# Validation-m3sSAGE/GCN_Recommendation

Measured on AMD Instinct MI355X. Metric: propagated edges/sec (SpMM) + Recall@20, Amazon-Books 3-layer d=64, higher is better.
Workload: dtype f32; 1 GPU; C3 full Amazon-Books-2023 shape (10.3M users x 4.4M items x 29.5M interactions); generator=powerlaw, users=10300000, items=4400000, interactions=29500000, nnz=56305746, d=64, layers=3, brands=0, content_dim=0, hub_threshold=128, hub_mode=exact, emu_min_degree=1024, parallelism=single

## Files before the change

### gcn_recommendation_amd/csrc/lgcn_engine.hip

```cpp
#include "lgcn_kernels.h"

#include <string.h>
#include <algorithm>
#include <functional>
#include <new>
#include <vector>

namespace lgcn_detail {
int g_rows_per_group = 0;
int g_unroll = 0;
int g_mean_prefetch = 0;
int g_min_groups = 0;
int g_emu_margin = (128 << 4) | 4;
int g_sample_blocks = 0;
int g_fusion_bwd_blocks = 0;
}

namespace {
__global__ void k_coo_inspect(const int64_t* __restrict__ rows, const int64_t* __restrict__ cols,
                              int64_t nnz, int32_t n_rows, int32_t n_cols, int32_t* flags) {
    const int64_t j = (int64_t)blockIdx.x * blockDim.x + threadIdx.x;
    if (j >= nnz) return;
    const int64_t r = rows[j], c = cols[j];
    int f = 0;
// ... 355 lines not shown

int scale_rows(const lgcn_rows_t& x, int32_t n_rows, int32_t d, float div, float* y, int64_t ldy,
               hipStream_t s) {
    const bool vec_ok = rows_aligned(x) && al16(y) && (ldy % 4 == 0);
    const Geo g = pick_geo(d, vec_ok);
    ScaleF f{&x, n_rows, g.dW, div, y, ldy, s};
    return dispatch_geo(g, f);
}

struct MeanEmptyF {
    const int32_t* row_ids; int32_t n; const lgcn_rows_t* e0; int32_t dW; float div;
    int32_t inv_bits; float* y; int64_t ldy; hipStream_t s;
    template <typename V, int G, int NV> int operator()() const {
        return launch_mean_empty_t<V, G, NV>(row_ids, n, *e0, dW, div, inv_bits, y, ldy, s);
    }
};

int mean_empty(const int32_t* row_ids, int32_t n, const lgcn_epilogue_t& ep_in, float* y,
               int64_t ldy, int32_t d, hipStream_t s) {
    const lgcn_epilogue_t ep = with_pow2(ep_in);
    const bool vec_ok = rows_aligned(ep.prev0) && al16(y) && (ldy % 4 == 0);
    const Geo g = pick_geo(d, vec_ok);
    MeanEmptyF f{row_ids, n, &ep.prev0, g.dW, ep.div, ep.pad, y, ldy, s};
    return dispatch_geo(g, f);
}

lgcn_rows_t dense_rows(const float* p, int32_t n, int64_t ld) {
    lgcn_rows_t r;
    r.p0 = r.p1 = r.p2 = p;
    r.end0 = r.end1 = n;
    r.ld = ld;
    return r;
}

int valid_geom(int32_t n_rows, int32_t d) {
    if (n_rows < 0 || d < 1 || d > 2048) return LGCN_EINVAL;
    return 0;
}

}

template <typename V>
__global__ __launch_bounds__(256) void k_add_nonzero(const V* __restrict__ src, V* __restrict__ dst,
                                                     int64_t m) {
    for (int64_t i = (int64_t)blockIdx.x * 256 + threadIdx.x; i < m;
         i += (int64_t)gridDim.x * 256) {
// ... 598 lines not shown
}

int link(const lgcn_sched* sc, hipStream_t from, hipStream_t to) {
    hipEvent_t e;
    if (int r = ev_next(sc, &e)) return r;
    if (int r = herr(hipEventRecord(e, from))) return r;
    return herr(hipStreamWaitEvent(to, e, 0));
}

int record(const lgcn_sched* sc, hipStream_t st, hipEvent_t* out) {
    if (int r = ev_next(sc, out)) return r;
    return herr(hipEventRecord(*out, st));
}

int wait_ev(hipStream_t st, hipEvent_t e) { return e ? herr(hipStreamWaitEvent(st, e, 0)) : 0; }

struct Deps {
    hipEvent_t late[3] = {nullptr, nullptr, nullptr};
    hipEvent_t late_emu[2] = {nullptr, nullptr};
    hipEvent_t part_wait[2] = {nullptr, nullptr};
    bool defer = false;
    hipEvent_t part_done[2] = {nullptr, nullptr};
    hipStream_t lk = nullptr;
};

int wait_late(hipStream_t st, const Deps* dp, bool emu = true) {
    if (!dp) return 0;
    for (hipEvent_t e : dp->late)
        if (int r = wait_ev(st, e)) return r;
    if (emu)
        for (hipEvent_t e : dp->late_emu)
            if (int r = wait_ev(st, e)) return r;
    return 0;
}

int part_blocks(const lgcn_edge_t* edges, const lgcn_hub_plan_t& p, const EmuPart& q,
                const lgcn_rows_t& x, float xdiv, const uint32_t* x_nz, int32_t d,
                const lgcn_emu_row_t* live, hipStream_t s) {
    if (q.b1 <= q.b0) return 0;
    const int64_t b0 = q.b0;
    return lgcn_emu_blocks(edges, p.emu_blocks + b0, q.b1 - q.b0, x, xdiv, x_nz, d,
                           p.emu_rel + b0 * d * LGCN_EMU_CANDS,
                           static_cast<char*>(p.emu_meta) + b0 * d * LGCN_EMU_META_BYTES,
                           p.emu_stage ? p.emu_stage + b0 * (d + 1) * LGCN_EMU_BLOCK : nullptr,
                           live, s);
}

// ... 10 lines not shown
bool chain_ok(const lgcn_rows_t& x, int32_t d) {
    return lgcn_chain_supported(d) && x.ld % 4 == 0 && al16(x.p0) && al16(x.p1) && al16(x.p2);
}

int plan_layer(const int32_t* rowptr, const lgcn_edge_t* edges, const int32_t* row_ids,
               int32_t n, const lgcn_hub_plan_t& p, const lgcn_rows_t& x, float xdiv,
               const uint32_t* x_nz, float* y, int64_t ldy, int32_t d, const lgcn_epilogue_t& ep,
               const lgcn_sched* sc, hipStream_t s, Deps* dp = nullptr) {
    const int32_t ne = p.n_emu_rows;
    const bool live = x_nz && p.emu_live && ne > 0 && chain_ok(x, d) && (!sc || sc->chain);
    const bool chains = !live && ne > p.emu_part_rows[1] && chain_ok(x, d) && (!sc || sc->chain);
    if ((chains || live ? p.emu_part_blocks[1] : p.n_emu_blocks) > p.emu_scratch_blocks)
        return LGCN_EINVAL;
    hipEvent_t* tr = sc ? sc->trace : nullptr;
    auto mark = [&](int k, hipStream_t st) -> int {
        return tr && tr[k] ? herr(hipEventRecord(tr[k], st)) : 0;
    };
    const EmuPart parts[3] = {{0, p.emu_part_rows[0], 0, p.emu_part_blocks[0]},
                              {p.emu_part_rows[0], p.emu_part_rows[1], p.emu_part_blocks[0],
                               p.emu_part_blocks[1]},
                              {p.emu_part_rows[1], ne, p.emu_part_blocks[1], p.n_emu_blocks}};
    const int slots[3] = {sc ? sc->slots[0] : 0, sc ? sc->slots[1] : 0, sc ? sc->slots[1] : 0};
    auto layer_kernel = [&](hipStream_t st) -> int {
        if (sc && sc->t0)
            if (int e = herr(hipEventRecord(sc->t0, st))) return e;
        if (int e = spmm_layer(rowptr, edges, row_ids, n, p.threshold, p.items, p.n_items,
                               p.partials, x, y, ldy, d, ep, xdiv, x_nz, st))
            return e;
        if (sc && sc->t1)
            if (int e = herr(hipEventRecord(sc->t1, st))) return e;
        return hub_combine(p.rows, p.n_rows, p.n_pre, p.partials, y, ldy, d, ep, st);
    };
    const bool has_late = dp && (dp->late[0] || dp->late[1] || dp->late[2] ||
                                 dp->late_emu[0] || dp->late_emu[1]);
    const bool defer_epi = sc && has_late && ep.mode == LGCN_EPI_MEAN && p.emu_out && ne > 0 &&
                           !live;
    lgcn_epilogue_t ep_rows;
    memset(&ep_rows, 0, sizeof(ep_rows));
    ep_rows.mode = LGCN_EPI_ROWS;
    auto emu_y = [&](int i) { return defer_epi ? p.emu_out + (int64_t)parts[i].r0 * d : y; };
    const int64_t emu_ld = defer_epi ? d : ldy;
    const lgcn_epilogue_t& emu_ep = defer_epi ? ep_rows : ep;
    auto chain_rows = [&](hipStream_t st) -> int {
        const EmuPart& q = parts[2];
        if (q.r1 <= q.r0) return 0;
        return lgcn_chain_rows(edges, p.emu_blocks, p.emu_rows + q.r0, q.r1 - q.r0, x, xdiv,
                               emu_y(2), emu_ld, d, &emu_ep, st);
    };
    const lgcn_emu_row_t* lflags =
        live ? lgcn_live_flags(p.emu_live, ne, p.n_emu_blocks) : nullptr;
    auto live_rows = [&](hipStream_t st) -> int {
        return lgcn_live_rows(edges, p.emu_blocks, p.n_emu_blocks, p.emu_rows, ne, x, xdiv, x_nz,
                              y, ldy, d, &ep, p.emu_part_rows[1], LGCN_LIVE_MAX, p.emu_live, st);
    };
// ... 208 lines not shown
    return 0;
}

bool classes_hold(const lgcn_sides_t& sd, const lgcn_hub_plan_t* plans) {
    for (int j = 0; j < 2; ++j) {
        const lgcn_hub_plan_t& p = plans[2 * 3 + j];
        if (p.emu_part_rows[0] > sd.part_rows[0] || p.emu_part_rows[1] > sd.part_rows[1])
            return false;
    }
    return true;
}

struct LayerIO {
    lgcn_rows_t x;
    float xdiv;
    const uint32_t* x_nz;
    float* y;
    lgcn_epilogue_t ep;
};

int seg_layer(const int32_t* rowptr, const lgcn_edge_t* edges, const int32_t* row_ids,
              int32_t lo, int32_t hi, const lgcn_hub_plan_t* plans, int k, int g,
              const LayerIO& io, int32_t d, const lgcn_sched* sc, const Lane& L, Deps* dp,
              int32_t empty_tail = 0) {
    if (empty_tail > 0) {
        hi -= empty_tail;
        if (io.ep.mode == LGCN_EPI_MEAN)
            if (int e = mean_empty(row_ids + hi, empty_tail, io.ep, io.y, d, d, L.main)) return e;
    }
    if (hi <= lo) {
        if (dp && dp->defer && sc)
            for (int i = 0; i < 2; ++i)
                if (int e = record(sc, L.main, &dp->part_done[i])) return e;
        return 0;
    }
    const int h = (k - 1) * kSegs + g;
    lgcn_sched v;
    const lgcn_sched* vp = nullptr;
    if (L.view) {
        v = *L.view;
        v.t0 = sc->timing_sides ? sc->timing_sides[2 * h] : nullptr;
        v.t1 = sc->timing_sides ? sc->timing_sides[2 * h + 1] : nullptr;
        v.trace = sc->trace_sides ? sc->trace_sides + h * 8 : nullptr;
        vp = &v;
    }
    Deps local;
    Deps* dq = dp;
    if (!vp && dp && dp->defer && sc) {
        local = *dp;
        local.defer = false;
        dq = &local;
    }
    if (int e = plan_layer(rowptr + lo, edges, row_ids + lo, hi - lo, plans[2 * g + (k & 1)],
                           io.x, io.xdiv, io.x_nz, io.y, d, d, io.ep, vp, L.main, dq))
        return e;
    if (dq == &local)
        for (int i = 0; i < 2; ++i)
            if (int e = record(sc, L.main, &dp->part_done[i])) return e;
    return 0;
}

int run_sides(const int32_t* rowptr, const lgcn_edge_t* edges, const int32_t* row_ids,
              const lgcn_sides_t& sd, const lgcn_hub_plan_t* plans, int32_t d, int32_t K,
              const std::function<LayerIO(int)>& layer, const lgcn_sched* sched, hipStream_t s,
              const int32_t* empty_tail = nullptr) {
    Lane lanes[2];
    bool l1_aux = false;
    if (sched) sched->pool->next = 0;
    const bool two = make_lanes(sched, s, lanes, l1_aux);
    const bool cap = capture_restricted(s);
    const bool classes = sched && sched->classes && classes_hold(sd, plans) && !cap;
    if (sched) sched->pool->state[3] = classes ? 1 : 0;
    const int32_t lo[kSegs] = {0, sd.class_end[0], sd.class_end[1], sd.split};
    const int32_t hi[kSegs] = {sd.class_end[0], sd.class_end[1], sd.split, 0};
    auto seg_hi = [&](int g, int32_t n) { return g == 3 ? n : hi[g]; };
    const int32_t n = sd.n;
    if (int e = fork_lanes(sched, two, lanes[1], s)) return e;
    constexpr int KM = LGCN_MAX_LAYERS + 2;
    hipEvent_t cls[KM][3] = {}, ab[KM] = {}, rest[KM] = {}, part[KM][2] = {};
    for (int k = 1; k <= K; ++k) {
        const LayerIO io = layer(k);
        const bool mean = io.ep.mode == LGCN_EPI_MEAN;
        {
            const Lane& L = lanes[(k + 1 + K) & 1];
            Deps dp;
            if (classes && k >= 2) {
                dp.part_wait[0] = cls[k - 1][0];
                dp.part_wait[1] = ab[k - 1];
            }
            dp.defer = k < K && sched && !cap;
            if (k == K && mean && sched && sched->lk_normal && two && l1_aux && !cap &&
                sched->n_aux >= 3)
                dp.lk = sched->aux[2];
            if (mean && k >= 2) {
                dp.late[0] = rest[k - 1];
                dp.late_emu[0] = part[k - 1][0];
                dp.late_emu[1] = part[k - 1][1];
            }
            if (int e = seg_layer(rowptr, edges, row_ids, sd.split, n, plans, k, 3, io, d, sched,
                                  L, &dp, empty_tail ? empty_tail[3] : 0))
                return e;
            if (k < K && sched) {
                if (int e = record(sched, L.main, &rest[k])) return e;
                part[k][0] = dp.part_done[0];
                part[k][1] = dp.part_done[1];
            }
        }
        {
            const Lane& L = lanes[(k + K) & 1];
            static const int up[3] = {0, 1, 2}, down[3] = {2, 1, 0};
            const int* order = k == 1 ? up : down;
            for (int t = 0; t < 3; ++t) {
                const int c = order[t];
                if (k >= 2 && (c <= 1 || !classes))
                    if (int e = wait_ev(L.main, part[k - 1][1])) return e;
                if (k >= 2 && (c == 0 || !classes))
                    if (int e = wait_ev(L.main, part[k - 1][0])) return e;
                Deps dp;
                if (mean && k >= 2) dp.late[0] = cls[k - 1][c];
                if (int e = seg_layer(rowptr, edges, row_ids, lo[c], seg_hi(c, n), plans, k, c,
                                      io, d, sched, L, &dp, empty_tail ? empty_tail[c] : 0))
                    return e;
                if (sched)
                    if (int e = record(sched, L.main, &cls[k][c])) return e;
            }
            ab[k] = k == 1 ? cls[k][1] : cls[k][0];
        }
    }
    return join_lanes(sched, two, lanes[1], s);
}
}

extern "C" {

int lgcn_sched_create(void* const* aux_streams, int32_t n_aux, lgcn_sched_t** out) {
    if (!out || n_aux < 1 || n_aux > 7 || !aux_streams) return LGCN_EINVAL;
    for (int i = 0; i < n_aux; ++i)
        if (!aux_streams[i]) return LGCN_EINVAL;
    lgcn_sched* sc = new (std::nothrow) lgcn_sched();
    EventPool* pool = new (std::nothrow) EventPool();
    if (!sc || !pool) {
        delete sc;
        delete pool;
        return LGCN_EINVAL;
// ... 152 lines not shown
            ep.prev0 = emb;
            for (int i = 0; i + 1 < K; ++i) ep.prev_dense[i] = layer_bufs_host[i];
            ep.ld_prev = d;
            y = out;
        }
        if (ev_host) {
            if (int e = herr(hipEventRecord((hipEvent_t)ev_host[2 * (k - 1)], s))) return e;
        }
        if (int e = plan_layer(rowptr, edges, row_ids, n, *plan, x, 1.f, nullptr, y, d, d, ep,
                               sched, s))
            return e;
        if (ev_host) {
            if (int e = herr(hipEventRecord((hipEvent_t)ev_host[2 * (k - 1) + 1], s))) return e;
        }
    }
    return 0;
}

int lgcn_propagate_forward_sides(const int32_t* rowptr, const lgcn_edge_t* edges,
                                 const int32_t* row_ids, const lgcn_sides_t* sides,
                                 const lgcn_hub_plan_t* plans, lgcn_rows_t emb, int32_t d,
                                 int32_t K, float* const* layer_bufs_host, float* out,
                                 const lgcn_sched_t* sched, void* stream) {
    return lgcn_propagate_forward_sides_lean(rowptr, edges, row_ids, sides, plans, nullptr, emb, d,
                                             K, layer_bufs_host, out, sched, stream);
}

int lgcn_propagate_forward_sides_lean(const int32_t* rowptr, const lgcn_edge_t* edges,
                                      const int32_t* row_ids, const lgcn_sides_t* sides,
                                      const lgcn_hub_plan_t* plans, const lgcn_lean_t* lean,
                                      lgcn_rows_t emb, int32_t d, int32_t K,
                                      float* const* layer_bufs_host, float* out,
                                      const lgcn_sched_t* sched, void* stream) {
    const int32_t n = sides ? sides->n : -1;
    if (int e = valid_geom(n, d)) return e;
    if (K < 0 || K - 1 > LGCN_MAX_LAYERS || !out) return K < 0 || !out ? LGCN_EINVAL : LGCN_ETOOMANY;
    if (K > 1 && !layer_bufs_host) return LGCN_EINVAL;
    hipStream_t s = S(stream);
    if (K == 0) return scale_rows(emb, n, d, 1.0f, out, d, s);
    if (int e = check_sides(rowptr, row_ids, n, sides, plans)) return e;
    auto layer = [&](int k) {
        LayerIO io;
        memset(&io, 0, sizeof(io));
        io.x = (k == 1) ? emb : dense_rows(layer_bufs_host[k - 2], n, d);
        io.xdiv = 1.f;
        if (k < K) {
            io.ep.mode = LGCN_EPI_STORE;
            io.y = layer_bufs_host[k - 1];
        } else {
            io.ep.mode = LGCN_EPI_MEAN;
            io.ep.n_prev = K;
            io.ep.div = (float)(K + 1);
            io.ep.prev0 = emb;
            for (int i = 0; i + 1 < K; ++i) io.ep.prev_dense[i] = layer_bufs_host[i];
            io.ep.ld_prev = d;
            io.y = out;
        }
        return io;
    };
    if (lean) {
        const int32_t b[kSegs + 1] = {0, sides->class_end[0], sides->class_end[1], sides->split, n};
        for (int g = 0; g < kSegs; ++g)
            if (lean->empty_tail[g] < 0 || lean->empty_tail[g] > b[g + 1] - b[g])
                return LGCN_EINVAL;
    }
    return run_sides(rowptr, edges, row_ids, *sides, plans, d, K, layer, sched, s,
                     lean ? lean->empty_tail : nullptr);
}

int lgcn_propagate_backward_sides(const int32_t* rowptr, const lgcn_edge_t* edges,
                                  const int32_t* row_ids, const lgcn_sides_t* sides,
                                  const lgcn_hub_plan_t* plans, lgcn_rows_t grad_out,
                                  const uint32_t* grad_nz, int32_t d, int32_t K, float* work_h,
                                  float* grad_e0, const lgcn_sched_t* sched, void* stream) {
    const int32_t n = sides ? sides->n : -1;
    if (int e = valid_geom(n, d)) return e;
    if (K < 0 || !grad_out.p0 || !grad_e0) return LGCN_EINVAL;
    hipStream_t s = S(stream);
    if (K == 0) return scale_rows(grad_out, n, d, 1.0f, grad_e0, d, s);
    if (K > 1 && !work_h) return LGCN_EINVAL;
    if (int e = check_sides(rowptr, row_ids, n, sides, plans)) return e;
    auto out_of = [&](int k) { return ((K - k) % 2 == 0) ? grad_e0 : work_h; };
    auto layer = [&](int k) {
        LayerIO io;
        memset(&io, 0, sizeof(io));
        io.x = k == 1 ? grad_out : dense_rows(out_of(k - 1), n, d);
        io.xdiv = k == 1 ? (float)(K + 1) : 1.f;
        io.x_nz = k == 1 ? grad_nz : nullptr;
        io.y = out_of(k);
        io.ep.mode = LGCN_EPI_ADD;
// ... 44 lines not shown
```

### gcn_recommendation_amd/csrc/lgcn_kernels.h

```cpp
#pragma once
#include <hip/hip_runtime.h>
#include <hipcub/hipcub.hpp>

#include <stdint.h>
#include <string.h>

#include "lgcn.h"


namespace lgcn_detail {
extern int g_rows_per_group;
extern int g_unroll;
extern int g_mean_prefetch;
extern int g_min_groups;

struct LayerArgs {
    const int32_t* rowptr;
    const lgcn_edge_t* edges;
    const int32_t* row_ids;
    int32_t n_rows, thr;
    const lgcn_hub_item_t* items;
    int32_t n_items;
    float* partials;
    lgcn_rows_t x;
// ... 536 lines not shown

template <typename V, int G, int NV>
__global__ __launch_bounds__(kBlock) void k_mean_empty(const int32_t* __restrict__ row_ids,
                                                       int32_t n_rows, lgcn_rows_t e0, int32_t dW,
                                                       float div, int32_t inv_bits,
                                                       float* __restrict__ y, int64_t ldy) {
    using T = VT<V>;
    constexpr int RPB = kBlock / G;
    const int lane = threadIdx.x & (G - 1);
    const int64_t slot = (int64_t)blockIdx.x * RPB + threadIdx.x / G;
    if (slot >= n_rows) return;
    const int32_t row = row_ids[slot];
    const float* xr = seg_row(e0, row);
#pragma unroll
    for (int q = 0; q < NV; ++q) {
        const int c = lane + q * G;
        if (c < dW)
            store_out<V>(y + (int64_t)row * ldy + c * T::W,
                         div_exact<V>(T::add(load_stream<V>(xr + c * T::W), T::zero()), div,
                                      inv_bits));
    }
}

template <typename V, int G, int NV>
__global__ __launch_bounds__(kBlock) void k_rows_nonzero(lgcn_rows_t x, int32_t n_rows, int32_t dW,
                                                         uint32_t* __restrict__ mask,
                                                         int32_t* __restrict__ count) {
    using T = VT<V>;
    constexpr int RPB = kBlock / G;
    constexpr int ROWS = 256;
    __shared__ uint32_t words[ROWS / 32];
    const int lane = threadIdx.x & (G - 1);
    const int grp = threadIdx.x / G;
    if (threadIdx.x < ROWS / 32) words[threadIdx.x] = 0;
    __syncthreads();
    const int64_t base = (int64_t)blockIdx.x * ROWS;
    for (int i = grp; i < ROWS; i += RPB) {
        const int64_t r = base + i;
        bool nz = false;
        if (r < n_rows) {
            const float* xr = seg_row(x, (int32_t)r);
#pragma unroll
            for (int q = 0; q < NV; ++q) {
                const int c = lane + q * G;
                if (c < dW) {
                    const V v = T::load(xr + c * T::W);
// ... 163 lines not shown
    }
    return last_err();
}

template <typename V, int G, int NV>
int launch_scale_t(const lgcn_rows_t& x, int32_t n_rows, int32_t dW, float div, float* y,
                   int64_t ldy, hipStream_t s) {
    constexpr int RPB = kBlock / G;
    const int64_t grid = ((int64_t)n_rows + RPB - 1) / RPB;
    if (grid == 0) return 0;
    hipLaunchKernelGGL((k_scale_rows<V, G, NV>), dim3((uint32_t)grid), dim3(kBlock), 0, s, x, n_rows,
                       dW, div, y, ldy);
    return last_err();
}

template <typename V, int G, int NV>
int launch_mean_empty_t(const int32_t* row_ids, int32_t n_rows, const lgcn_rows_t& e0, int32_t dW,
                        float div, int32_t inv_bits, float* y, int64_t ldy, hipStream_t s) {
    constexpr int RPB = kBlock / G;
    const int64_t grid = ((int64_t)n_rows + RPB - 1) / RPB;
    if (grid == 0) return 0;
    hipLaunchKernelGGL((k_mean_empty<V, G, NV>), dim3((uint32_t)grid), dim3(kBlock), 0, s, row_ids,
                       n_rows, e0, dW, div, inv_bits, y, ldy);
    return last_err();
}

template <typename F>
int dispatch_geo(const Geo& g, const F& f) {
#define LGCN_CASE(VT_, G_, NV_) \
    if (g.G == G_ && g.NV == NV_) return f.template operator()<VT_, G_, NV_>();
    if (g.vec) {
        LGCN_CASE(float4, 4, 1)
        LGCN_CASE(float4, 8, 1)
        LGCN_CASE(float4, 16, 1)
        LGCN_CASE(float4, 32, 1)
        LGCN_CASE(float4, 64, 1)
        LGCN_CASE(float4, 64, 2)
        LGCN_CASE(float4, 64, 4)
        LGCN_CASE(float4, 64, 8)
    } else {
        LGCN_CASE(float, 4, 1)
        LGCN_CASE(float, 8, 1)
        LGCN_CASE(float, 16, 1)
        LGCN_CASE(float, 32, 1)
        LGCN_CASE(float, 64, 1)
        LGCN_CASE(float, 64, 2)
// ... 28 lines not shown
```

### gcn_recommendation_amd/engine.py

```python
import ctypes
import os
import threading

import numpy as np
import torch

_PKG = os.path.dirname(os.path.abspath(__file__))
LIB_PATH = os.path.join(_PKG, "liblgcn_engine.so")

LGCN_EPI_STORE, LGCN_EPI_MEAN, LGCN_EPI_ADD = 0, 1, 2
LGCN_SCATTER_STORE, LGCN_SCATTER_ADD = 0, 1
LGCN_MAX_LAYERS = 16
COO_ROWS_UNSORTED, COO_OUT_OF_RANGE, COO_COLS_UNSORTED = 1, 2, 4
INT32_MAX = 2 ** 31 - 1
TUNE_ROWS_PER_GROUP, TUNE_UNROLL, TUNE_MEAN_PREFETCH, TUNE_MIN_GROUPS = 1, 2, 3, 4
TUNE_EMU_MARGIN = 6
TUNE_SAMPLE_BLOCKS = 7
TUNE_FUSION_BWD_BLOCKS = 8
FUSION_BWD_CHUNK = 2048
SCHED_SLOTS0, SCHED_SLOTS1, SCHED_CHAIN, SCHED_TIMING_START, SCHED_TIMING_END, SCHED_TRACE = \
    1, 2, 3, 4, 5, 6
SCHED_TRACE_SIDES, SCHED_TIMING_SIDES = 7, 8
SCHED_CLASSES = 16
SCHED_LK_NORMAL = 17
# ... 59 lines not shown
                ("addend", RowsT), ("addend_nz", ctypes.c_void_p)]


class PlanT(ctypes.Structure):
    _fields_ = [("items", ctypes.c_void_p), ("rows", ctypes.c_void_p), ("partials", ctypes.c_void_p),
                ("emu_blocks", ctypes.c_void_p), ("emu_rows", ctypes.c_void_p),
                ("emu_rel", ctypes.c_void_p), ("emu_meta", ctypes.c_void_p),
                ("emu_stage", ctypes.c_void_p),
                ("threshold", ctypes.c_int32), ("n_items", ctypes.c_int32),
                ("n_rows", ctypes.c_int32), ("n_pre", ctypes.c_int32),
                ("n_emu_blocks", ctypes.c_int32), ("n_emu_rows", ctypes.c_int32),
                ("emu_part_rows", ctypes.c_int32 * 2), ("emu_part_blocks", ctypes.c_int32 * 2),
                ("emu_scratch_blocks", ctypes.c_int32), ("emu_live", ctypes.c_void_p),
                ("emu_part_max_blocks", ctypes.c_int32 * 2), ("emu_out", ctypes.c_void_p)]


class SidesT(ctypes.Structure):
    _fields_ = [("n", ctypes.c_int32), ("split", ctypes.c_int32), ("class_end", ctypes.c_int32 * 2),
                ("part_rows", ctypes.c_int32 * 2)]


class LeanT(ctypes.Structure):
    _fields_ = [("empty_tail", ctypes.c_int32 * 4)]


class LgcnError(RuntimeError):
    pass


_lib = None
_lib_lock = threading.Lock()

_P, _I32, _I64 = ctypes.c_void_p, ctypes.c_int32, ctypes.c_int64
ABI = [
    ("lgcn_abi_version", ctypes.c_int, []),
    ("lgcn_error_string", ctypes.c_char_p, [ctypes.c_int]),
    ("lgcn_tune", ctypes.c_int, [ctypes.c_int, ctypes.c_int]),
    ("lgcn_device_info", ctypes.c_int, [ctypes.c_int, _P, _P]),
    ("lgcn_stream_create", ctypes.c_int, [_I32, _P]),
    ("lgcn_capture_full_schedule", ctypes.c_int, []),
    ("lgcn_stream_destroy", ctypes.c_int, [_P]),
    ("lgcn_coo_inspect", ctypes.c_int, [_P, _P, _I64, _I32, _I32, _P, _P]),
    ("lgcn_coo_to_csr", ctypes.c_int, [_P, _P, _P, _I64, _I32, _P, _P, _P, _P, _P]),
    ("lgcn_coo_sort_perm", ctypes.c_int, [_P, _I64, _I32, _P, _P, _P, _P, _P,
                                          ctypes.POINTER(ctypes.c_size_t), _P]),
    ("lgcn_csr_check_symmetric", ctypes.c_int, [_P, _P, _I32, _I64, _P, _P]),
# ... 63 lines not shown
    ("lgcn_live_scratch_bytes", ctypes.c_size_t, [_I32, _I32]),
    ("lgcn_live_rows", ctypes.c_int, [_P, _P, _I32, _P, _I32, RowsT, ctypes.c_float, _P, _P, _I64,
                                      _I32, ctypes.POINTER(EpilogueT), _I32, _I32, _P, _P]),
    ("lgcn_live_flags", ctypes.c_void_p, [_P, _I32, _I32]),
    ("lgcn_chain_rows", ctypes.c_int, [_P, _P, _P, _I32, RowsT, ctypes.c_float, _P, _I64, _I32,
                                       ctypes.POINTER(EpilogueT), _P]),
    ("lgcn_sched_create", ctypes.c_int, [_P, _I32, ctypes.POINTER(ctypes.c_void_p)]),
    ("lgcn_sched_destroy", ctypes.c_int, [_P]),
    ("lgcn_sched_set", ctypes.c_int, [_P, _I32, _I64]),
    ("lgcn_sched_state", ctypes.c_int64, [_P, _I32]),
    ("lgcn_layer", ctypes.c_int, [_P, _P, _P, _I32, ctypes.POINTER(PlanT), RowsT, ctypes.c_float, _P,
                                  _P, _I64, _I32, ctypes.POINTER(EpilogueT), _P, _P]),
    ("lgcn_propagate_forward", ctypes.c_int, [_P, _P, _P, _I32, ctypes.POINTER(PlanT), RowsT, _I32,
                                              _I32, _P, _P, _P, _P, _P]),
    ("lgcn_propagate_backward", ctypes.c_int, [_P, _P, _P, _I32, ctypes.POINTER(PlanT), RowsT, _P,
                                               _I32, _I32, _P, _P, _P, _P]),
    ("lgcn_propagate_forward_sides", ctypes.c_int, [_P, _P, _P, ctypes.POINTER(SidesT),
                                                    ctypes.POINTER(PlanT), RowsT, _I32, _I32, _P,
                                                    _P, _P, _P]),
    ("lgcn_propagate_forward_sides_lean", ctypes.c_int, [_P, _P, _P, ctypes.POINTER(SidesT),
                                                         ctypes.POINTER(PlanT),
                                                         ctypes.POINTER(LeanT), RowsT, _I32, _I32,
                                                         _P, _P, _P, _P]),
    ("lgcn_propagate_backward_sides", ctypes.c_int, [_P, _P, _P, ctypes.POINTER(SidesT),
                                                     ctypes.POINTER(PlanT), RowsT, _P, _I32, _I32,
                                                     _P, _P, _P, _P]),
]


def load_library(path=None):
    global _lib
    with _lib_lock:
        if _lib is not None:
            return _lib
        p = path or os.environ.get("LGCN_LIB") or LIB_PATH
        if not os.path.exists(p):
            raise LgcnError(f"liblgcn_engine.so not found at {p}: run `python -c \"import "
                            f"__graft_entry__ as g; g.build()\"` (hipcc --offload-arch=gfx950)")
        lib = ctypes.CDLL(p)
        for name, res, args in ABI:
            fn = getattr(lib, name)
            fn.restype = res
            fn.argtypes = args
        if lib.lgcn_abi_version() != ABI_VERSION:
            raise LgcnError("liblgcn_engine.so ABI version mismatch")
        _lib = lib
# ... 360 lines not shown
    def n_derived(self):
        return self.lean().n_derived

    def degrees(self):
        deg = np.diff(self.rowptr_host().astype(np.int64))
        ids = self.row_ids_host()
        if ids is None:
            return deg
        out = np.empty_like(deg)
        out[ids] = deg
        return out


def _bitmask(flags):
    n = flags.numel()
    pad = torch.zeros(((n + 31) // 32) * 32, dtype=torch.int64, device=flags.device)
    pad[:n] = flags
    w = (pad.view(-1, 32) << torch.arange(32, dtype=torch.int64, device=flags.device)).sum(1)
    return torch.where(w >= 1 << 31, w - (1 << 32), w).to(torch.int32)


class LeanPlan:

    def __init__(self, empty, derived, n_empty, n_derived, empty_tail):
        self.empty, self.derived = empty, derived
        self.n_empty, self.n_derived = n_empty, n_derived
        self.empty_tail = tuple(empty_tail)

    def struct(self):
        st = LeanT()
        for g, t in enumerate(self.empty_tail):
            st.empty_tail[g] = t
        return st


def lean_plan(rowptr, edges, row_ids, split, segments):
    dev = rowptr.device
    n = rowptr.numel() - 1
    nnz = int(rowptr[-1])
    ids = row_ids.long()
    deg_slot = (rowptr[1:] - rowptr[:-1]).long()
    rec = edges[:nnz]
    col = rec & 0xffffffff
    bits = rec >> 32
    row = torch.repeat_interleave(ids, deg_slot)
    deg = torch.zeros(n, dtype=torch.int64, device=dev)
    deg[ids] = deg_slot
    named = torch.zeros(n, dtype=torch.bool, device=dev)
    named[col] = True
    empty = (deg == 0) & ~named
    one_slot = deg_slot == 1
    first = rec[rowptr[:-1].long()[one_slot]]
    p = torch.full((n,), -1, dtype=torch.int64, device=dev)
    w = torch.zeros(n, dtype=torch.int64, device=dev)
    p[ids[one_slot]] = first & 0xffffffff
    w[ids[one_slot]] = first >> 32
    side0 = torch.zeros(n, dtype=torch.bool, device=dev)
    side0[ids[:split]] = True
    other = torch.zeros(n, dtype=torch.bool, device=dev)
    other[col[(row != p[col]) | (bits != w[col])]] = True
    derived = (deg == 1) & side0 & ~other
    tails = []
    for a, b in segments:
        e = empty[ids[a:b]]
        live = torch.nonzero(~e)
        tails.append(int(b - a - (int(live[-1]) + 1 if live.numel() else 0)))
    return LeanPlan(_bitmask(empty), _bitmask(derived), int(empty.sum()), int(derived.sum()),
                    tails)


def slot_key_enabled(g):
    return g.n_rows == g.n_cols and os.environ.get("LGCN_SLOT_KEY", "1") != "0"


def order_by_degree(lib, g, stream, sides=None):
    n, nnz, dev = g.n_rows, g.nnz, g.device
    lo, hi = sides if sides is not None else (0, 0)
    i32 = dict(dtype=torch.int32, device=dev)
    deg_tmp, deg_sorted, iota = (torch.empty(max(n, 1), **i32) for _ in range(3))
    row_ids = torch.empty(max(n, 1), **i32)
    rowptr = torch.empty(n + 1, **i32)
    edges = torch.empty(max(nnz, 1), dtype=torch.int64, device=dev)
    keys = (torch.empty(max(n, 1), dtype=torch.int64, device=dev) for _ in range(2)) \
        if slot_key_enabled(g) else (None, None)
    key_tmp, key_sorted = keys
    nbytes = ctypes.c_size_t(0)
    args = (_ptr(g.rowptr), _ptr(g.edges), n, nnz, lo, hi, _ptr(deg_tmp), _ptr(deg_sorted),
            _ptr(iota),
            _ptr(row_ids), _ptr(rowptr), _ptr(edges),
            _ptr(key_tmp) if key_tmp is not None else None,
            _ptr(key_sorted) if key_sorted is not None else None)
    _check(lib.lgcn_csr_order_by_degree(*args, None, ctypes.byref(nbytes), stream),
           "lgcn_csr_order_by_degree(size)")
    temp = torch.empty(max(nbytes.value, 1), dtype=torch.uint8, device=dev)
    _check(lib.lgcn_csr_order_by_degree(*args, _ptr(temp), ctypes.byref(nbytes), stream),
           "lgcn_csr_order_by_degree")
    del deg_tmp, deg_sorted, iota, temp, key_tmp, key_sorted
    o = Graph(n, g.n_cols, rowptr, edges, nnz, dev, row_ids=row_ids[:n])
    o.symmetric = g.symmetric
    if lo < hi:
        o.sides, o.split = (lo, hi), n - (hi - lo)
        if classes_enabled():
            o = side_classes(lib, o, stream)
    return o


def classes_enabled():
    return os.environ.get("LGCN_CLASSES", "0") == "1"


PART0_SPARSE_BACKWARD = 2048


def walk_cut_blocks(nnz, backward=False, part0=None):
    b1 = -(-chain_max_degree(nnz, backward) // LGCN_EMU_BLOCK)
    b0 = int(os.environ.get("LGCN_EMU_PART0", "") or part0 or 8192)
    return max(b0, b1), b1


def side_classes(lib, g, stream):
    n, nnz, dev, sp = g.n_rows, g.nnz, g.device, g.split
    b0, b1 = walk_cut_blocks(nnz)
    deg1 = np.diff(g.rowptr_host()[sp:].astype(np.int64))
    nb = -(-deg1 // LGCN_EMU_BLOCK)
    p0, p01 = int((nb > b0).sum()), int((nb > b1).sum())
    if p01 == 0 or sp == 0:
# ... 409 lines not shown
def use_sides(graph, layer_events=None, kernel_events=None):
    return graph.split is not None and layer_events is None and kernel_events is None


def _collect_sides(ev, K, graph):
    segs = [g for g, (a, b) in enumerate(graph.segments()) if b > a]
    if ev.timing is not None and side_timing is not None:
        side_timing.append({(k, g): (ev.timing[((k - 1) * N_SEGS + g) * 2],
                                     ev.timing[((k - 1) * N_SEGS + g) * 2 + 1])
                            for k in range(1, K + 1) for g in segs})
    if ev.trace is not None and side_trace is not None:
        side_trace.append({(k, g): list(zip(TRACE_PHASES,
                                            ev.trace[((k - 1) * N_SEGS + g) * 8:
                                                     ((k - 1) * N_SEGS + g + 1) * 8]))
                           for k in range(1, K + 1) for g in segs})


def alloc_layers(n, d, count, device):
    return [torch.empty((n, d), dtype=torch.float32, device=device) for _ in range(count)]


def propagate_forward(graph, segments, K, hub_threshold=None, layer_events=None,
                      return_layers=False, hub_mode=None, emu_min=None, kernel_events=None,
                      lean=None):
    if hub_threshold is None:
        hub_threshold = hub_threshold_from_env()
    d = segments[0].shape[1]
    n = sum(int(t.shape[0]) for t in segments)
    if n != graph.n_rows:
        raise LgcnError(f"embedding rows {n} != adjacency size {graph.n_rows}")
    _check_emb(segments, d, graph.device)
    if K > LGCN_MAX_LAYERS + 1 or K < 0:
        raise LgcnError(f"n_layers={K} unsupported (0..{LGCN_MAX_LAYERS + 1})")
    lib = load_library()
    dev = graph.device
    with torch.cuda.device(dev):
        stream = _stream(dev)
        e0 = rows_desc(segments, d)
        out = torch.empty((n, d), dtype=torch.float32, device=dev)
        if K == 0:
            _check(lib.lgcn_scale_rows(e0, n, d, 1.0, _ptr(out), d, stream), "lgcn_scale_rows")
            return (out, []) if return_layers else out
        layers = alloc_layers(n, d, K - 1, dev)
        if use_sides(graph, layer_events, kernel_events):
            if lean is None:
                lean = not return_layers
            lp = graph.lean().struct() if lean else None
            plans, _ = _side_plans(graph, d, hub_threshold, hub_mode, emu_min,
                                   _aligned16(segments))
            sc = sched_for(dev)
            ev = _SideEvents(sc, K, side_timing is not None, side_trace is not None)
            bufs = (ctypes.c_void_p * max(K - 1, 1))(*[t.data_ptr() for t in layers])
            sides = graph.sides_struct()
            try:
                _check(lib.lgcn_propagate_forward_sides_lean(
                    _ptr(graph.rowptr), _ptr(graph.edges), _ptr(graph.row_ids),
                    ctypes.byref(sides), plans, ctypes.byref(lp) if lp is not None else None,
                    e0, d, K, bufs, _ptr(out),
                    sc.handle if sc is not None else None, stream),
                    "lgcn_propagate_forward_sides_lean")
            finally:
                ev.clear()
            _note_schedule(sc, graph)
            _collect_sides(ev, K, graph)
            return (out, layers) if return_layers else out
        hp = graph.hubs(hub_threshold, mode=hub_mode, emu_min=emu_min)
        for k in range(1, K + 1):
            xs = segments if k == 1 else [layers[k - 2]]
            if k < K:
                y, ep = layers[k - 1], _epilogue(LGCN_EPI_STORE)
            else:
                y = out
                ep = _epilogue(LGCN_EPI_MEAN, prev0=e0, prev_dense=layers, ld_prev=d,
                               div=float(K + 1))
            if layer_events is not None:
                layer_events[k - 1][0].record()
            spmm_layer(graph, xs, y, d, ep, hub_threshold, hp, stream,
                       kernel_events=None if kernel_events is None else kernel_events[k - 1])
            if layer_events is not None:
                layer_events[k - 1][1].record()
        return (out, layers) if return_layers else out


# ... 240 lines not shown
```

### include/lgcn.h

```cpp
#ifndef LGCN_H_
#define LGCN_H_

#include <stdint.h>
#include <stddef.h>

#ifdef __cplusplus
extern "C" {
#endif

#define LGCN_ABI_VERSION 14

#define LGCN_EINVAL      (-1)
#define LGCN_EALIGN      (-2)
#define LGCN_ETOOMANY    (-3)

#define LGCN_MAX_LAYERS 16

#define LGCN_COO_ROWS_UNSORTED   1
#define LGCN_COO_OUT_OF_RANGE    2
#define LGCN_COO_COLS_UNSORTED   4

#define LGCN_EPI_STORE 0
#define LGCN_EPI_MEAN  1
#define LGCN_EPI_ADD   2
// ... 240 lines not shown
                            const uint32_t* grad_nz, int32_t d, int32_t K, float* work_h,
                            float* grad_e0, const lgcn_sched_t* sched, void* stream);

typedef struct {
    int32_t n;
    int32_t split;
    int32_t class_end[2];
    int32_t part_rows[2];
} lgcn_sides_t;
int lgcn_propagate_forward_sides(const int32_t* rowptr, const lgcn_edge_t* edges,
                                 const int32_t* row_ids, const lgcn_sides_t* sides,
                                 const lgcn_hub_plan_t* plans, lgcn_rows_t emb, int32_t d,
                                 int32_t K, float* const* layer_bufs_host, float* out,
                                 const lgcn_sched_t* sched, void* stream);
typedef struct {
    int32_t empty_tail[4];
} lgcn_lean_t;
int lgcn_propagate_forward_sides_lean(const int32_t* rowptr, const lgcn_edge_t* edges,
                                      const int32_t* row_ids, const lgcn_sides_t* sides,
                                      const lgcn_hub_plan_t* plans, const lgcn_lean_t* lean,
                                      lgcn_rows_t emb, int32_t d, int32_t K,
                                      float* const* layer_bufs_host, float* out,
                                      const lgcn_sched_t* sched, void* stream);
int lgcn_propagate_backward_sides(const int32_t* rowptr, const lgcn_edge_t* edges,
                                  const int32_t* row_ids, const lgcn_sides_t* sides,
                                  const lgcn_hub_plan_t* plans, lgcn_rows_t grad_out,
                                  const uint32_t* grad_nz, int32_t d, int32_t K, float* work_h,
                                  float* grad_e0, const lgcn_sched_t* sched, void* stream);

int lgcn_bpr_loss(const float* u, int64_t ldu, const float* p, int64_t ldp, const float* n,
                  int64_t ldn, const float* u0, int64_t ldu0, const float* p0, int64_t ldp0,
                  const float* n0, int64_t ldn0, int32_t B, int32_t d, float lambda, float* terms,
                  float* loss, float* grads, void* stream);

int lgcn_bpr_loss_indexed(const float* fu, int64_t ld_fu, const float* fi, int64_t ld_fi,
                          const float* u0, int64_t ld_u0, const float* i0, int64_t ld_i0,
                          int64_t n_users, int64_t n_items, const int64_t* users,
                          const int64_t* pos, const int64_t* neg, int32_t B, int32_t d,
                          float lambda, float* terms, float* loss, float* grads, void* stream);

int lgcn_bpr_keys(const int64_t* users, const int64_t* pos, const int64_t* neg, int32_t B,
                  int64_t n_users, int64_t n_items, int64_t* keys, void* stream);

#define LGCN_SCATTER_STORE 0
#define LGCN_SCATTER_ADD   1
int lgcn_rows_scatter(const int32_t* keys_sorted, const int32_t* perm, int32_t n, const float* src,
// ... 74 lines not shown
```

Baseline: 14.95 billion edges/s.

## Alias degree-one rows sharing a neighbor and compute their final mean on a side stream

Finds degree-1 derived rows whose single neighbor is the same record, keeps one representative, and moves the aliased rows to the segment tail. Later layers store only the representative's layer values, and other-side edges are remapped to the representative through a second edge array. A new mean_shared kernel builds the final-layer mean for the aliased rows from the representative's stored layers, overlapped on an auxiliary stream. The goal is to skip redundant SpMM work for duplicated rows, at the cost of graph reordering at build time, an extra remapped edge array and more complex scheduling.

```diff
diff --git a/gcn_recommendation_amd/csrc/lgcn_engine.hip b/gcn_recommendation_amd/csrc/lgcn_engine.hip
--- a/gcn_recommendation_amd/csrc/lgcn_engine.hip
+++ b/gcn_recommendation_amd/csrc/lgcn_engine.hip
@@ -401,6 +401,26 @@
     const bool vec_ok = rows_aligned(ep.prev0) && al16(y) && (ldy % 4 == 0);
     const Geo g = pick_geo(d, vec_ok);
     MeanEmptyF f{row_ids, n, &ep.prev0, g.dW, ep.div, ep.pad, y, ldy, s};
+    return dispatch_geo(g, f);
+}
+
+struct MeanSharedF {
+    const int32_t* rowptr; const lgcn_edge_t* edges; const int32_t* row_ids;
+    const int32_t* rep_of; int32_t n; const lgcn_rows_t* x; int32_t dW;
+    const lgcn_epilogue_t* ep; float* y; int64_t ldy; hipStream_t s;
+    template <typename V, int G, int NV> int operator()() const {
+        return launch_mean_shared_t<V, G, NV>(rowptr, edges, row_ids, rep_of, n, *x, dW, *ep, y,
+                                              ldy, s);
+    }
+};
+
+int mean_shared(const int32_t* rowptr, const lgcn_edge_t* edges, const int32_t* row_ids,
+                const int32_t* rep_of, int32_t n, const lgcn_rows_t& x,
+                const lgcn_epilogue_t& ep_in, float* y, int64_t ldy, int32_t d, hipStream_t s) {
+    const lgcn_epilogue_t ep = with_pow2(ep_in);
+    const bool vec_ok = rows_aligned(x) && al16(y) && (ldy % 4 == 0) && epi_aligned(ep);
+    const Geo g = pick_geo(d, vec_ok);
+    MeanSharedF f{rowptr, edges, row_ids, rep_of, n, &x, g.dW, &ep, y, ldy, s};
     return dispatch_geo(g, f);
 }
 
@@ -1045,7 +1065,10 @@
     bool defer = false;
     hipEvent_t part_done[2] = {nullptr, nullptr};
     hipStream_t lk = nullptr;
+    std::function<int(hipStream_t)> pre;
 };
+
+bool capture_restricted(hipStream_t s);
 
 int wait_late(hipStream_t st, const Deps* dp, bool emu = true) {
     if (!dp) return 0;
@@ -1102,6 +1125,15 @@
                               {p.emu_part_rows[1], ne, p.emu_part_blocks[1], p.n_emu_blocks}};
     const int slots[3] = {sc ? sc->slots[0] : 0, sc ? sc->slots[1] : 0, sc ? sc->slots[1] : 0};
     auto layer_kernel = [&](hipStream_t st) -> int {
+        hipStream_t side = nullptr;
+        if (dp && dp->pre) {
+            const int ax = sc ? (sc->n_aux > 1 ? 1 : 0) : 0;
+            if (sc && sc->n_aux > 0 && sc->aux[ax] != st && !capture_restricted(st)) {
+                side = sc->aux[ax];
+                if (int e = link(sc, st, side)) return e;
+            }
+            if (int e = dp->pre(side ? side : st)) return e;
+        }
         if (sc && sc->t0)
             if (int e = herr(hipEventRecord(sc->t0, st))) return e;
         if (int e = spmm_layer(rowptr, edges, row_ids, n, p.threshold, p.items, p.n_items,
@@ -1109,7 +1141,8 @@
             return e;
         if (sc && sc->t1)
             if (int e = herr(hipEventRecord(sc->t1, st))) return e;
-        return hub_combine(p.rows, p.n_rows, p.n_pre, p.partials, y, ldy, d, ep, st);
+        if (int e = hub_combine(p.rows, p.n_rows, p.n_pre, p.partials, y, ldy, d, ep, st)) return e;
+        return side ? link(sc, side, st) : 0;
     };
     const bool has_late = dp && (dp->late[0] || dp->late[1] || dp->late[2] ||
                                  dp->late_emu[0] || dp->late_emu[1]);
@@ -1364,11 +1397,30 @@
 int seg_layer(const int32_t* rowptr, const lgcn_edge_t* edges, const int32_t* row_ids,
               int32_t lo, int32_t hi, const lgcn_hub_plan_t* plans, int k, int g,
               const LayerIO& io, int32_t d, const lgcn_sched* sc, const Lane& L, Deps* dp,
-              int32_t empty_tail = 0) {
+              int32_t empty_tail = 0, int32_t shared_tail = 0,
+              const int32_t* rep_of = nullptr) {
     if (empty_tail > 0) {
         hi -= empty_tail;
         if (io.ep.mode == LGCN_EPI_MEAN)
             if (int e = mean_empty(row_ids + hi, empty_tail, io.ep, io.y, d, d, L.main)) return e;
+    }
+    if (shared_tail > 0) {
+        if (!dp || !rep_of) return LGCN_EINVAL;
+        const int32_t first = hi - shared_tail;
+        if (io.ep.mode == LGCN_EPI_MEAN) {
+            const LayerIO lio = io;
+            auto pre = [=](hipStream_t st) {
+                return mean_shared(rowptr + first, edges, row_ids + first, rep_of, shared_tail,
+                                   lio.x, lio.ep, lio.y, d, d, st);
+            };
+            if (first <= lo) {
+                if (int e = wait_late(L.main, dp)) return e;
+                if (int e = pre(L.main)) return e;
+            } else {
+                dp->pre = pre;
+            }
+        }
+        hi -= shared_tail;
     }
     if (hi <= lo) {
         if (dp && dp->defer && sc)
@@ -1405,7 +1457,8 @@
 int run_sides(const int32_t* rowptr, const lgcn_edge_t* edges, const int32_t* row_ids,
               const lgcn_sides_t& sd, const lgcn_hub_plan_t* plans, int32_t d, int32_t K,
               const std::function<LayerIO(int)>& layer, const lgcn_sched* sched, hipStream_t s,
-              const int32_t* empty_tail = nullptr) {
+              const int32_t* empty_tail = nullptr, const lgcn_shared_t* sh = nullptr) {
+    const lgcn_edge_t* edges1 = sh ? sh->edges1 - sh->edges1_first : edges;
     Lane lanes[2];
     bool l1_aux = false;
     if (sched) sched->pool->next = 0;
@@ -1439,8 +1492,8 @@
                 dp.late_emu[0] = part[k - 1][0];
                 dp.late_emu[1] = part[k - 1][1];
             }
-            if (int e = seg_layer(rowptr, edges, row_ids, sd.split, n, plans, k, 3, io, d, sched,
-                                  L, &dp, empty_tail ? empty_tail[3] : 0))
+            if (int e = seg_layer(rowptr, k >= 2 ? edges1 : edges, row_ids, sd.split, n, plans, k,
+                                  3, io, d, sched, L, &dp, empty_tail ? empty_tail[3] : 0))
                 return e;
             if (k < K && sched) {
                 if (int e = record(sched, L.main, &rest[k])) return e;
@@ -1461,7 +1514,8 @@
                 Deps dp;
                 if (mean && k >= 2) dp.late[0] = cls[k - 1][c];
                 if (int e = seg_layer(rowptr, edges, row_ids, lo[c], seg_hi(c, n), plans, k, c,
-                                      io, d, sched, L, &dp, empty_tail ? empty_tail[c] : 0))
+                                      io, d, sched, L, &dp, empty_tail ? empty_tail[c] : 0,
+                                      sh ? sh->shared_tail[c] : 0, sh ? sh->rep_of : nullptr))
                     return e;
                 if (sched)
                     if (int e = record(sched, L.main, &cls[k][c])) return e;
@@ -1660,8 +1714,9 @@
                                  const lgcn_hub_plan_t* plans, lgcn_rows_t emb, int32_t d,
                                  int32_t K, float* const* layer_bufs_host, float* out,
                                  const lgcn_sched_t* sched, void* stream) {
-    return lgcn_propagate_forward_sides_lean(rowptr, edges, row_ids, sides, plans, nullptr, emb, d,
-                                             K, layer_bufs_host, out, sched, stream);
+    return lgcn_propagate_forward_sides_shared(rowptr, edges, row_ids, sides, plans, nullptr,
+                                               nullptr, emb, d, K, layer_bufs_host, out, sched,
+                                               stream);
 }
 
 int lgcn_propagate_forward_sides_lean(const int32_t* rowptr, const lgcn_edge_t* edges,
@@ -1670,6 +1725,16 @@
                                       lgcn_rows_t emb, int32_t d, int32_t K,
                                       float* const* layer_bufs_host, float* out,
                                       const lgcn_sched_t* sched, void* stream) {
+    return lgcn_propagate_forward_sides_shared(rowptr, edges, row_ids, sides, plans, lean, nullptr,
+                                               emb, d, K, layer_bufs_host, out, sched, stream);
+}
+
+int lgcn_propagate_forward_sides_shared(const int32_t* rowptr, const lgcn_edge_t* edges,
+                                        const int32_t* row_ids, const lgcn_sides_t* sides,
+                                        const lgcn_hub_plan_t* plans, const lgcn_lean_t* lean,
+                                        const lgcn_shared_t* shared, lgcn_rows_t emb, int32_t d,
+                                        int32_t K, float* const* layer_bufs_host, float* out,
+                                        const lgcn_sched_t* sched, void* stream) {
     const int32_t n = sides ? sides->n : -1;
     if (int e = valid_geom(n, d)) return e;
     if (K < 0 || K - 1 > LGCN_MAX_LAYERS || !out) return K < 0 || !out ? LGCN_EINVAL : LGCN_ETOOMANY;
@@ -1702,8 +1767,21 @@
             if (lean->empty_tail[g] < 0 || lean->empty_tail[g] > b[g + 1] - b[g])
                 return LGCN_EINVAL;
     }
+    if (shared && (K < 2 || !(shared->shared_tail[0] | shared->shared_tail[1] |
+                              shared->shared_tail[2] | shared->shared_tail[3])))
+        shared = nullptr;
+    if (shared) {
+        if (!lean || !shared->rep_of || !shared->edges1 || shared->edges1_first < 0 ||
+            shared->shared_tail[3] != 0)
+            return LGCN_EINVAL;
+        const int32_t b[kSegs] = {0, sides->class_end[0], sides->class_end[1], sides->split};
+        for (int g = 0; g < 3; ++g)
+            if (shared->shared_tail[g] < 0 ||
+                shared->shared_tail[g] > b[g + 1] - b[g] - lean->empty_tail[g])
+                return LGCN_EINVAL;
+    }
     return run_sides(rowptr, edges, row_ids, *sides, plans, d, K, layer, sched, s,
-                     lean ? lean->empty_tail : nullptr);
+                     lean ? lean->empty_tail : nullptr, shared);
 }
 
 int lgcn_propagate_backward_sides(const int32_t* rowptr, const lgcn_edge_t* edges,
diff --git a/gcn_recommendation_amd/csrc/lgcn_kernels.h b/gcn_recommendation_amd/csrc/lgcn_kernels.h
--- a/gcn_recommendation_amd/csrc/lgcn_kernels.h
+++ b/gcn_recommendation_amd/csrc/lgcn_kernels.h
@@ -582,6 +582,64 @@
     }
 }
 
+template <typename V, int G, int NV, int U, int NP>
+__global__ __launch_bounds__(kBlock) void k_mean_shared(const int32_t* __restrict__ rowptr,
+                                                        const lgcn_edge_t* __restrict__ edges,
+                                                        const int32_t* __restrict__ row_ids,
+                                                        const int32_t* __restrict__ rep_of,
+                                                        int32_t n_rows, lgcn_rows_t x, int32_t dW,
+                                                        lgcn_epilogue_t ep, float* __restrict__ y,
+                                                        int64_t ldy) {
+    using T = VT<V>;
+    constexpr int RPB = kBlock / G;
+    const int lane = threadIdx.x & (G - 1);
+    const int64_t slot = (int64_t)blockIdx.x * RPB + threadIdx.x / G;
+    if (slot >= n_rows) return;
+    const int32_t beg = rowptr[slot];
+    const int32_t end = rowptr[slot + 1];
+    const int32_t row = row_ids[slot];
+    const int32_t rep = rep_of[row];
+    V acc[NV];
+#pragma unroll
+    for (int q = 0; q < NV; ++q) acc[q] = T::zero();
+    float* yr = y + (int64_t)row * ldy;
+    if constexpr (NP > 0) {
+        V pre[NP][NV];
+#pragma unroll
+        for (int p = 0; p < NP; ++p) {
+            const float* src = p == 0 ? seg_row(ep.prev0, row)
+                                      : ep.prev_dense[p - 1] + (int64_t)rep * ep.ld_prev;
+#pragma unroll
+            for (int q = 0; q < NV; ++q) {
+                const int c = lane + q * G;
+                pre[p][q] = c < dW ? load_stream<V>(src + c * T::W) : T::zero();
+            }
+        }
+        accumulate<V, G, NV, U, 0>(edges, beg, end, x, lane, dW, acc);
+#pragma unroll
+        for (int q = 0; q < NV; ++q) {
+            const int c = lane + q * G;
+            if (c >= dW) continue;
+            V s = pre[0][q];
+#pragma unroll
+            for (int p = 1; p < NP; ++p) s = T::add(s, pre[p][q]);
+            store_out<V>(yr + c * T::W, div_exact<V>(T::add(s, acc[q]), ep.div, ep.pad));
+        }
+    } else {
+        accumulate<V, G, NV, U, 0>(edges, beg, end, x, lane, dW, acc);
+#pragma unroll
+        for (int q = 0; q < NV; ++q) {
+            const int c = lane + q * G;
+            if (c >= dW) continue;
+            V s = load_stream<V>(seg_row(ep.prev0, row) + c * T::W);
+            for (int i = 0; i + 1 < ep.n_prev; ++i)
+                s = T::add(s, load_stream<V>(ep.prev_dense[i] + (int64_t)rep * ep.ld_prev + c * T::W));
+            s = T::add(s, acc[q]);
+            store_out<V>(yr + c * T::W, div_exact<V>(s, ep.div, ep.pad));
+        }
+    }
+}
+
 template <typename V, int G, int NV>
 __global__ __launch_bounds__(kBlock) void k_rows_nonzero(lgcn_rows_t x, int32_t n_rows, int32_t dW,
                                                          uint32_t* __restrict__ mask,
@@ -791,6 +849,25 @@
     if (grid == 0) return 0;
     hipLaunchKernelGGL((k_mean_empty<V, G, NV>), dim3((uint32_t)grid), dim3(kBlock), 0, s, row_ids,
                        n_rows, e0, dW, div, inv_bits, y, ldy);
+    return last_err();
+}
+
+template <typename V, int G, int NV>
+int launch_mean_shared_t(const int32_t* rowptr, const lgcn_edge_t* edges, const int32_t* row_ids,
+                         const int32_t* rep_of, int32_t n_rows, const lgcn_rows_t& x, int32_t dW,
+                         const lgcn_epilogue_t& ep, float* y, int64_t ldy, hipStream_t s) {
+    constexpr int RPB = kBlock / G;
+    constexpr int U1 = NV >= 8 ? 1 : 8 / NV;
+    const int64_t grid = ((int64_t)n_rows + RPB - 1) / RPB;
+    if (grid == 0) return 0;
+#define LGCN_LAUNCH(NP_)                                                                          \
+    hipLaunchKernelGGL((k_mean_shared<V, G, NV, U1, NP_>), dim3((uint32_t)grid), dim3(kBlock), 0, \
+                       s, rowptr, edges, row_ids, rep_of, n_rows, x, dW, ep, y, ldy)
+    if (NV <= 2 && ep.n_prev == 2) LGCN_LAUNCH(2);
+    else if (NV <= 2 && ep.n_prev == 3) LGCN_LAUNCH(3);
+    else if (NV <= 2 && ep.n_prev == 4) LGCN_LAUNCH(4);
+    else LGCN_LAUNCH(0);
+#undef LGCN_LAUNCH
     return last_err();
 }
 
diff --git a/gcn_recommendation_amd/engine.py b/gcn_recommendation_amd/engine.py
--- a/gcn_recommendation_amd/engine.py
+++ b/gcn_recommendation_amd/engine.py
@@ -105,6 +105,11 @@
 
 class LeanT(ctypes.Structure):
     _fields_ = [("empty_tail", ctypes.c_int32 * 4)]
+
+
+class SharedT(ctypes.Structure):
+    _fields_ = [("shared_tail", ctypes.c_int32 * 4), ("rep_of", ctypes.c_void_p),
+                ("edges1", ctypes.c_void_p), ("edges1_first", ctypes.c_int64)]
 
 
 class LgcnError(RuntimeError):
@@ -214,6 +219,11 @@
                                                          ctypes.POINTER(PlanT),
                                                          ctypes.POINTER(LeanT), RowsT, _I32, _I32,
                                                          _P, _P, _P, _P]),
+    ("lgcn_propagate_forward_sides_shared", ctypes.c_int, [_P, _P, _P, ctypes.POINTER(SidesT),
+                                                           ctypes.POINTER(PlanT),
+                                                           ctypes.POINTER(LeanT),
+                                                           ctypes.POINTER(SharedT), RowsT, _I32,
+                                                           _I32, _P, _P, _P, _P]),
     ("lgcn_propagate_backward_sides", ctypes.c_int, [_P, _P, _P, ctypes.POINTER(SidesT),
                                                      ctypes.POINTER(PlanT), RowsT, _P, _I32, _I32,
                                                      _P, _P, _P, _P]),
@@ -620,10 +630,14 @@
 
 class LeanPlan:
 
-    def __init__(self, empty, derived, n_empty, n_derived, empty_tail):
+    def __init__(self, empty, derived, n_empty, n_derived, empty_tail, rep_of=None,
+                 shared_tail=(0, 0, 0, 0), edges1=None, edges1_first=0):
         self.empty, self.derived = empty, derived
         self.n_empty, self.n_derived = n_empty, n_derived
         self.empty_tail = tuple(empty_tail)
+        self.rep_of, self.edges1, self.edges1_first = rep_of, edges1, int(edges1_first)
+        self.shared_tail = tuple(shared_tail)
+        self.n_shared = sum(self.shared_tail)
 
     def struct(self):
         st = LeanT()
@@ -631,8 +645,18 @@
             st.empty_tail[g] = t
         return st
 
-
-def lean_plan(rowptr, edges, row_ids, split, segments):
+    def shared_struct(self):
+        if self.n_shared == 0:
+            return None
+        st = SharedT()
+        for g, t in enumerate(self.shared_tail):
+            st.shared_tail[g] = t
+        st.rep_of, st.edges1 = self.rep_of.data_ptr(), self.edges1.data_ptr()
+        st.edges1_first = self.edges1_first
+        return st
+
+
+def _lean_masks(rowptr, edges, row_ids, split):
     dev = rowptr.device
     n = rowptr.numel() - 1
     nnz = int(rowptr[-1])
@@ -658,13 +682,75 @@
     other = torch.zeros(n, dtype=torch.bool, device=dev)
     other[col[(row != p[col]) | (bits != w[col])]] = True
     derived = (deg == 1) & side0 & ~other
-    tails = []
-    for a, b in segments:
-        e = empty[ids[a:b]]
-        live = torch.nonzero(~e)
-        tails.append(int(b - a - (int(live[-1]) + 1 if live.numel() else 0)))
+    return empty, derived, side0, ids, deg_slot, rec
+
+
+def _empty_tail(empty, ids, a, b):
+    live = torch.nonzero(~empty[ids[a:b]])
+    return int(b - a - (int(live[-1]) + 1 if live.numel() else 0))
+
+
+def _shared_groups(rowptr, rec, ids, deg_slot, derived, side0, a, b):
+    at = torch.nonzero(deg_slot[a:b] == 1).flatten()
+    if at.numel() == 0 or int(at[-1]) - int(at[0]) + 1 != at.numel():
+        return None
+    lo, hi = a + int(at[0]), a + int(at[-1]) + 1
+    rows = ids[lo:hi]
+    recs = rec[rowptr[lo:hi].long()]
+    member = derived[rows] & ~side0[recs & 0xffffffff]
+    pos = torch.nonzero(member).flatten()
+    alias = torch.zeros_like(member)
+    rep = rows.clone()
+    if pos.numel():
+        _, inv = torch.unique(recs[pos], return_inverse=True)
+        first = torch.full((int(inv.max()) + 1,), hi, dtype=torch.int64, device=rows.device)
+        first.scatter_reduce_(0, inv, pos, "amin")
+        alias[pos] = pos != first[inv]
+        rep[pos] = rows[first[inv]]
+    return lo, hi, rows, recs, alias, rep
+
+
+def shared_rows_order(rowptr, edges, row_ids, split, segments):
+    empty, derived, side0, ids, deg_slot, rec = _lean_masks(rowptr, edges, row_ids, split)
+    moved = 0
+    for a, b in segments[:3]:
+        gr = _shared_groups(rowptr, rec, ids, deg_slot, derived, side0, a, b) if b > a else None
+        if gr is None:
+            continue
+        lo, hi, rows, recs, alias, _ = gr
+        if hi != b - _empty_tail(empty, ids, a, b) or not bool(alias.any()):
+            continue
+        perm = torch.cat([torch.nonzero(~alias).flatten(), torch.nonzero(alias).flatten()])
+        row_ids[lo:hi] = rows[perm].to(row_ids.dtype)
+        edges[rowptr[lo:hi].long()] = recs[perm]
+        moved += int(alias.sum())
+    return moved
+
+
+def lean_plan(rowptr, edges, row_ids, split, segments):
+    dev = rowptr.device
+    n = rowptr.numel() - 1
+    empty, derived, side0, ids, deg_slot, rec = _lean_masks(rowptr, edges, row_ids, split)
+    tails = [_empty_tail(empty, ids, a, b) for a, b in segments]
+    rep_of = torch.arange(n, dtype=torch.int32, device=dev)
+    shared = [0, 0, 0, 0]
+    for g, (a, b) in enumerate(segments[:3]):
+        gr = _shared_groups(rowptr, rec, ids, deg_slot, derived, side0, a, b) if b > a else None
+        if gr is None:
+            continue
+        lo, hi, rows, _, alias, rep = gr
+        cnt = int(alias.sum())
+        if cnt == 0 or hi != b - tails[g] or not bool(alias[hi - lo - cnt:].all()):
+            continue
+        shared[g] = cnt
+        rep_of[rows[alias]] = rep[alias].to(torch.int32)
+    edges1, first1 = None, 0
+    if sum(shared):
+        first1 = int(rowptr[split])
+        rec1 = rec[first1:]
+        edges1 = (rec1 & ~0xffffffff) | rep_of[rec1 & 0xffffffff].long()
     return LeanPlan(_bitmask(empty), _bitmask(derived), int(empty.sum()), int(derived.sum()),
-                    tails)
+                    tails, rep_of, shared, edges1, first1)
 
 
 def slot_key_enabled(g):
@@ -700,6 +786,8 @@
         o.sides, o.split = (lo, hi), n - (hi - lo)
         if classes_enabled():
             o = side_classes(lib, o, stream)
+        if o.split > 0 and nnz > 0:
+            shared_rows_order(o.rowptr, o.edges, o.row_ids, o.split, o.segments())
     return o
 
 
@@ -1155,7 +1243,7 @@
 
 def propagate_forward(graph, segments, K, hub_threshold=None, layer_events=None,
                       return_layers=False, hub_mode=None, emu_min=None, kernel_events=None,
-                      lean=None):
+                      lean=None, shared=None):
     if hub_threshold is None:
         hub_threshold = hub_threshold_from_env()
     d = segments[0].shape[1]
@@ -1178,7 +1266,12 @@
         if use_sides(graph, layer_events, kernel_events):
             if lean is None:
                 lean = not return_layers
+            if shared is None:
+                shared = lean and not return_layers
+            if shared and not lean:
+                raise LgcnError("shared=True needs the lean forward (lean=True)")
             lp = graph.lean().struct() if lean else None
+            sp = graph.lean().shared_struct() if shared else None
             plans, _ = _side_plans(graph, d, hub_threshold, hub_mode, emu_min,
                                    _aligned16(segments))
             sc = sched_for(dev)
@@ -1186,12 +1279,13 @@
             bufs = (ctypes.c_void_p * max(K - 1, 1))(*[t.data_ptr() for t in layers])
             sides = graph.sides_struct()
             try:
-                _check(lib.lgcn_propagate_forward_sides_lean(
+                _check(lib.lgcn_propagate_forward_sides_shared(
                     _ptr(graph.rowptr), _ptr(graph.edges), _ptr(graph.row_ids),
                     ctypes.byref(sides), plans, ctypes.byref(lp) if lp is not None else None,
+                    ctypes.byref(sp) if sp is not None else None,
                     e0, d, K, bufs, _ptr(out),
                     sc.handle if sc is not None else None, stream),
-                    "lgcn_propagate_forward_sides_lean")
+                    "lgcn_propagate_forward_sides_shared")
             finally:
                 ev.clear()
             _note_schedule(sc, graph)
diff --git a/include/lgcn.h b/include/lgcn.h
--- a/include/lgcn.h
+++ b/include/lgcn.h
@@ -286,6 +286,18 @@
                                       lgcn_rows_t emb, int32_t d, int32_t K,
                                       float* const* layer_bufs_host, float* out,
                                       const lgcn_sched_t* sched, void* stream);
+typedef struct {
+    int32_t shared_tail[4];
+    const int32_t* rep_of;
+    const lgcn_edge_t* edges1;
+    int64_t edges1_first;
+} lgcn_shared_t;
+int lgcn_propagate_forward_sides_shared(const int32_t* rowptr, const lgcn_edge_t* edges,
+                                        const int32_t* row_ids, const lgcn_sides_t* sides,
+                                        const lgcn_hub_plan_t* plans, const lgcn_lean_t* lean,
+                                        const lgcn_shared_t* shared, lgcn_rows_t emb, int32_t d,
+                                        int32_t K, float* const* layer_bufs_host, float* out,
+                                        const lgcn_sched_t* sched, void* stream);
 int lgcn_propagate_backward_sides(const int32_t* rowptr, const lgcn_edge_t* edges,
                                   const int32_t* row_ids, const lgcn_sides_t* sides,
                                   const lgcn_hub_plan_t* plans, lgcn_rows_t grad_out,
```

After: 14.99 billion edges/s, median of 6. No clear change (+0.3%).
